# jjery2243542/adaptive_voice_conversion

Measured on NVIDIA H100. Metric: mel-segments/sec (80x128) train step, higher is better.
Workload: dtype tf32

## Files before the change

### adaptive_voice_conversion_b200/csrc/tc_common.cuh

```cuda
#pragma once
#include <cuda_runtime.h>
#include <stdint.h>

namespace avc {
namespace tc {

__device__ __forceinline__ uint32_t smem_u32(const void* p) { return (uint32_t)__cvta_generic_to_shared(p); }

__device__ __forceinline__ void mbar_init(uint64_t* bar, uint32_t count) {
  asm volatile("mbarrier.init.shared::cta.b64 [%0], %1;" ::"r"(smem_u32(bar)), "r"(count) : "memory");
}
__device__ __forceinline__ void fence_mbar_init() { asm volatile("fence.mbarrier_init.release.cluster;" ::: "memory"); }
__device__ __forceinline__ void mbar_arrive(uint64_t* bar) {
  asm volatile("mbarrier.arrive.shared::cta.b64 _, [%0];" ::"r"(smem_u32(bar)) : "memory");
}
__device__ __forceinline__ void mbar_arrive_expect_tx(uint64_t* bar, uint32_t bytes) {
  asm volatile("mbarrier.arrive.expect_tx.shared::cta.b64 _, [%0], %1;" ::"r"(smem_u32(bar)), "r"(bytes) : "memory");
}
__device__ __forceinline__ bool mbar_try_wait(uint64_t* bar, uint32_t parity) {
  uint32_t ok;
  asm volatile(
      "{\n\t.reg .pred p;\n\t"
      "mbarrier.try_wait.parity.shared::cta.b64 p, [%1], %2;\n\t"
      "selp.u32 %0, 1, 0, p;\n\t}"
// ... 45 lines not shown
}
__device__ __forceinline__ int warp_idx_sync() { return __shfl_sync(0xffffffffu, (int)(threadIdx.x >> 5), 0); }

template <int R>
__device__ __forceinline__ void setmaxnreg_dec() { asm volatile("setmaxnreg.dec.sync.aligned.u32 %0;" ::"n"(R)); }
template <int R>
__device__ __forceinline__ void setmaxnreg_inc() { asm volatile("setmaxnreg.inc.sync.aligned.u32 %0;" ::"n"(R)); }

__device__ __forceinline__ void wgmma_fence() { asm volatile("wgmma.fence.sync.aligned;" ::: "memory"); }
__device__ __forceinline__ void wgmma_commit() { asm volatile("wgmma.commit_group.sync.aligned;" ::: "memory"); }
template <int N>
__device__ __forceinline__ void wgmma_wait() { asm volatile("wgmma.wait_group.sync.aligned %0;" ::"n"(N) : "memory"); }
__device__ __forceinline__ void acc_fence(float* d, int n) {
  for (int i = 0; i < n; ++i) asm volatile("" : "+f"(d[i])::"memory");
}

template <int N>
__device__ __forceinline__ void wgmma_tf32(float* d, uint64_t a, uint64_t b, uint32_t acc);
template <> __device__ __forceinline__ void wgmma_tf32<16>(float* d, uint64_t a, uint64_t b, uint32_t acc) {
  asm volatile("{\n\t.reg .pred p;\n\tsetp.ne.b32 p, %10, 0;\n\t"
               "wgmma.mma_async.sync.aligned.m64n16k8.f32.tf32.tf32 {%0, %1, %2, %3, %4, %5, %6, %7}, %8, %9, p, 1, 1;\n\t}"
               : "+f"(d[0]), "+f"(d[1]), "+f"(d[2]), "+f"(d[3]), "+f"(d[4]), "+f"(d[5]), "+f"(d[6]), "+f"(d[7])
               : "l"(a), "l"(b), "r"(acc));
}
template <> __device__ __forceinline__ void wgmma_tf32<32>(float* d, uint64_t a, uint64_t b, uint32_t acc) {
  asm volatile("{\n\t.reg .pred p;\n\tsetp.ne.b32 p, %18, 0;\n\t"
               "wgmma.mma_async.sync.aligned.m64n32k8.f32.tf32.tf32 {%0, %1, %2, %3, %4, %5, %6, %7, %8, %9, %10, %11, %12, %13, %14, %15}, %16, %17, p, 1, 1;\n\t}"
               : "+f"(d[0]), "+f"(d[1]), "+f"(d[2]), "+f"(d[3]), "+f"(d[4]), "+f"(d[5]), "+f"(d[6]), "+f"(d[7]), "+f"(d[8]), "+f"(d[9]), "+f"(d[10]), "+f"(d[11]), "+f"(d[12]), "+f"(d[13]), "+f"(d[14]), "+f"(d[15])
               : "l"(a), "l"(b), "r"(acc));
}
// ... 70 lines not shown
               : "l"(a), "l"(b), "r"(acc));
}
template <> __device__ __forceinline__ void wgmma_tf32<240>(float* d, uint64_t a, uint64_t b, uint32_t acc) {
  asm volatile("{\n\t.reg .pred p;\n\tsetp.ne.b32 p, %122, 0;\n\t"
               "wgmma.mma_async.sync.aligned.m64n240k8.f32.tf32.tf32 {%0, %1, %2, %3, %4, %5, %6, %7, %8, %9, %10, %11, %12, %13, %14, %15, %16, %17, %18, %19, %20, %21, %22, %23, %24, %25, %26, %27, %28, %29, %30, %31, %32, %33, %34, %35, %36, %37, %38, %39, %40, %41, %42, %43, %44, %45, %46, %47, %48, %49, %50, %51, %52, %53, %54, %55, %56, %57, %58, %59, %60, %61, %62, %63, %64, %65, %66, %67, %68, %69, %70, %71, %72, %73, %74, %75, %76, %77, %78, %79, %80, %81, %82, %83, %84, %85, %86, %87, %88, %89, %90, %91, %92, %93, %94, %95, %96, %97, %98, %99, %100, %101, %102, %103, %104, %105, %106, %107, %108, %109, %110, %111, %112, %113, %114, %115, %116, %117, %118, %119}, %120, %121, p, 1, 1;\n\t}"
               : "+f"(d[0]), "+f"(d[1]), "+f"(d[2]), "+f"(d[3]), "+f"(d[4]), "+f"(d[5]), "+f"(d[6]), "+f"(d[7]), "+f"(d[8]), "+f"(d[9]), "+f"(d[10]), "+f"(d[11]), "+f"(d[12]), "+f"(d[13]), "+f"(d[14]), "+f"(d[15]), "+f"(d[16]), "+f"(d[17]), "+f"(d[18]), "+f"(d[19]), "+f"(d[20]), "+f"(d[21]), "+f"(d[22]), "+f"(d[23]), "+f"(d[24]), "+f"(d[25]), "+f"(d[26]), "+f"(d[27]), "+f"(d[28]), "+f"(d[29]), "+f"(d[30]), "+f"(d[31]), "+f"(d[32]), "+f"(d[33]), "+f"(d[34]), "+f"(d[35]), "+f"(d[36]), "+f"(d[37]), "+f"(d[38]), "+f"(d[39]), "+f"(d[40]), "+f"(d[41]), "+f"(d[42]), "+f"(d[43]), "+f"(d[44]), "+f"(d[45]), "+f"(d[46]), "+f"(d[47]), "+f"(d[48]), "+f"(d[49]), "+f"(d[50]), "+f"(d[51]), "+f"(d[52]), "+f"(d[53]), "+f"(d[54]), "+f"(d[55]), "+f"(d[56]), "+f"(d[57]), "+f"(d[58]), "+f"(d[59]), "+f"(d[60]), "+f"(d[61]), "+f"(d[62]), "+f"(d[63]), "+f"(d[64]), "+f"(d[65]), "+f"(d[66]), "+f"(d[67]), "+f"(d[68]), "+f"(d[69]), "+f"(d[70]), "+f"(d[71]), "+f"(d[72]), "+f"(d[73]), "+f"(d[74]), "+f"(d[75]), "+f"(d[76]), "+f"(d[77]), "+f"(d[78]), "+f"(d[79]), "+f"(d[80]), "+f"(d[81]), "+f"(d[82]), "+f"(d[83]), "+f"(d[84]), "+f"(d[85]), "+f"(d[86]), "+f"(d[87]), "+f"(d[88]), "+f"(d[89]), "+f"(d[90]), "+f"(d[91]), "+f"(d[92]), "+f"(d[93]), "+f"(d[94]), "+f"(d[95]), "+f"(d[96]), "+f"(d[97]), "+f"(d[98]), "+f"(d[99]), "+f"(d[100]), "+f"(d[101]), "+f"(d[102]), "+f"(d[103]), "+f"(d[104]), "+f"(d[105]), "+f"(d[106]), "+f"(d[107]), "+f"(d[108]), "+f"(d[109]), "+f"(d[110]), "+f"(d[111]), "+f"(d[112]), "+f"(d[113]), "+f"(d[114]), "+f"(d[115]), "+f"(d[116]), "+f"(d[117]), "+f"(d[118]), "+f"(d[119])
               : "l"(a), "l"(b), "r"(acc));
}
template <> __device__ __forceinline__ void wgmma_tf32<256>(float* d, uint64_t a, uint64_t b, uint32_t acc) {
  asm volatile("{\n\t.reg .pred p;\n\tsetp.ne.b32 p, %130, 0;\n\t"
               "wgmma.mma_async.sync.aligned.m64n256k8.f32.tf32.tf32 {%0, %1, %2, %3, %4, %5, %6, %7, %8, %9, %10, %11, %12, %13, %14, %15, %16, %17, %18, %19, %20, %21, %22, %23, %24, %25, %26, %27, %28, %29, %30, %31, %32, %33, %34, %35, %36, %37, %38, %39, %40, %41, %42, %43, %44, %45, %46, %47, %48, %49, %50, %51, %52, %53, %54, %55, %56, %57, %58, %59, %60, %61, %62, %63, %64, %65, %66, %67, %68, %69, %70, %71, %72, %73, %74, %75, %76, %77, %78, %79, %80, %81, %82, %83, %84, %85, %86, %87, %88, %89, %90, %91, %92, %93, %94, %95, %96, %97, %98, %99, %100, %101, %102, %103, %104, %105, %106, %107, %108, %109, %110, %111, %112, %113, %114, %115, %116, %117, %118, %119, %120, %121, %122, %123, %124, %125, %126, %127}, %128, %129, p, 1, 1;\n\t}"
               : "+f"(d[0]), "+f"(d[1]), "+f"(d[2]), "+f"(d[3]), "+f"(d[4]), "+f"(d[5]), "+f"(d[6]), "+f"(d[7]), "+f"(d[8]), "+f"(d[9]), "+f"(d[10]), "+f"(d[11]), "+f"(d[12]), "+f"(d[13]), "+f"(d[14]), "+f"(d[15]), "+f"(d[16]), "+f"(d[17]), "+f"(d[18]), "+f"(d[19]), "+f"(d[20]), "+f"(d[21]), "+f"(d[22]), "+f"(d[23]), "+f"(d[24]), "+f"(d[25]), "+f"(d[26]), "+f"(d[27]), "+f"(d[28]), "+f"(d[29]), "+f"(d[30]), "+f"(d[31]), "+f"(d[32]), "+f"(d[33]), "+f"(d[34]), "+f"(d[35]), "+f"(d[36]), "+f"(d[37]), "+f"(d[38]), "+f"(d[39]), "+f"(d[40]), "+f"(d[41]), "+f"(d[42]), "+f"(d[43]), "+f"(d[44]), "+f"(d[45]), "+f"(d[46]), "+f"(d[47]), "+f"(d[48]), "+f"(d[49]), "+f"(d[50]), "+f"(d[51]), "+f"(d[52]), "+f"(d[53]), "+f"(d[54]), "+f"(d[55]), "+f"(d[56]), "+f"(d[57]), "+f"(d[58]), "+f"(d[59]), "+f"(d[60]), "+f"(d[61]), "+f"(d[62]), "+f"(d[63]), "+f"(d[64]), "+f"(d[65]), "+f"(d[66]), "+f"(d[67]), "+f"(d[68]), "+f"(d[69]), "+f"(d[70]), "+f"(d[71]), "+f"(d[72]), "+f"(d[73]), "+f"(d[74]), "+f"(d[75]), "+f"(d[76]), "+f"(d[77]), "+f"(d[78]), "+f"(d[79]), "+f"(d[80]), "+f"(d[81]), "+f"(d[82]), "+f"(d[83]), "+f"(d[84]), "+f"(d[85]), "+f"(d[86]), "+f"(d[87]), "+f"(d[88]), "+f"(d[89]), "+f"(d[90]), "+f"(d[91]), "+f"(d[92]), "+f"(d[93]), "+f"(d[94]), "+f"(d[95]), "+f"(d[96]), "+f"(d[97]), "+f"(d[98]), "+f"(d[99]), "+f"(d[100]), "+f"(d[101]), "+f"(d[102]), "+f"(d[103]), "+f"(d[104]), "+f"(d[105]), "+f"(d[106]), "+f"(d[107]), "+f"(d[108]), "+f"(d[109]), "+f"(d[110]), "+f"(d[111]), "+f"(d[112]), "+f"(d[113]), "+f"(d[114]), "+f"(d[115]), "+f"(d[116]), "+f"(d[117]), "+f"(d[118]), "+f"(d[119]), "+f"(d[120]), "+f"(d[121]), "+f"(d[122]), "+f"(d[123]), "+f"(d[124]), "+f"(d[125]), "+f"(d[126]), "+f"(d[127])
               : "l"(a), "l"(b), "r"(acc));
}

__device__ __forceinline__ int wg_acc_row(int t, int i) { return 16 * (t >> 5) + ((t & 31) >> 2) + ((i & 2) ? 8 : 0); }
__device__ __forceinline__ int wg_acc_col(int t, int i) { return 8 * (i >> 2) + 2 * (t & 3) + (i & 1); }

}
}
```

### adaptive_voice_conversion_b200/csrc/wgrad_tc.cu

```cuda
#include "common.cuh"
#include "tc_common.cuh"

namespace avc {

constexpr int WT_NT = 32;
constexpr int WG_ROWS = 32;
constexpr int WG_A_BYTES = (WG_ROWS / 4) * 128 * 16;
constexpr int WG_MAX_STAGES = 8;
constexpr int WG_SMEM_MAX = 224 * 1024;

struct WgTcArgs {
  avc_wgrad_desc d;
  float* scratch;
  int nslices, samp_per_slice, nstage, coutp;
  int* status;
};

__device__ __forceinline__ float comp4(const float4& v, int c) { return c == 0 ? v.x : c == 1 ? v.y : c == 2 ? v.z : v.w; }

struct WgJob {
  float4 v[4];
  uint32_t dst;
  int rot;
};

template <int K>
__device__ __forceinline__ WgJob wgrad_job_load(const WgTcArgs& a, int e, int ch, int b0, int R) {
  const avc_wgrad_desc& d = a.d;
  const int T = d.Tout;
  WgJob J;
  const bool is_dc = e < 256;
  const int f = is_dc ? e : e - 256;
  const int c4 = is_dc ? (f & 31) : (f & 7), pl = is_dc ? (f >> 5) : ((f >> 3) & 7), j = is_dc ? 0 : (f >> 6);
  const int r = ch * WG_ROWS + 4 * pl;
  const int g = r / T, t = r - g * T;
  J.rot = (c4 >> 1) & 3;
  if (is_dc) {
    J.dst = (uint32_t)pl * (128u * 16u) + (uint32_t)(4 * c4) * 16u;
    const int co = blockIdx.y * 128 + 4 * c4;
    if (r < R && co < d.Cout) {
      const float* src = d.dc + (size_t)(b0 + g) * d.dc_bstride + ((size_t)(co >> 2) * T + t) * 4;
#pragma unroll
      for (int i = 0; i < 4; ++i) J.v[i] = ldg4(src + 4 * i);
    } else {
#pragma unroll
      for (int i = 0; i < 4; ++i) J.v[i] = zero4();
    }
  } else {
    J.dst = (uint32_t)WG_A_BYTES + (uint32_t)pl * (uint32_t)(K * WT_NT * 16) + (uint32_t)(j * WT_NT + 4 * c4) * 16u;
    const int ci = blockIdx.x * WT_NT + 4 * c4;
    const bool v = r < R && ci < d.Cin;
    const float* col = d.x + (size_t)(v ? b0 + g : 0) * d.x_bstride + (size_t)((v ? ci : 0) >> 2) * d.Tin * 4;
#pragma unroll
    for (int i = 0; i < 4; ++i) {
      const int p = src_pos((t + i) * d.stride + j - d.pad_left, d.Tin, AVC_PAD_REFLECT, 1);
      J.v[i] = (v && p >= 0) ? ldg4(col + (size_t)p * 4) : zero4();
    }
  }
  return J;
}

__device__ __forceinline__ void wgrad_job_store(uint8_t* stage, const WgJob& J) {
#pragma unroll
  for (int k = 0; k < 4; ++k) {
    const int c = (k + J.rot) & 3;
    *reinterpret_cast<float4*>(stage + J.dst + (uint32_t)c * 16u) = make_float4(comp4(J.v[0], c), comp4(J.v[1], c), comp4(J.v[2], c), comp4(J.v[3], c));
  }
}

__host__ __device__ constexpr int wg_stagers(int K) { return K <= 5 ? 2 : 1; }
__host__ __device__ constexpr int wg_threads(int K) { return 128 * (wg_stagers(K) + 2); }

template <int K, bool ATOMIC>
__global__ void __launch_bounds__(wg_threads(K), 1) conv_wgrad_wgmma_kernel(const WgTcArgs a) {
  constexpr int STAGERS = wg_stagers(K);
  constexpr int N = K * WT_NT;
  constexpr uint32_t B_PLANE = N * 16;
  extern __shared__ __align__(1024) uint8_t smem[];
  __shared__ uint64_t bar_full[WG_MAX_STAGES], bar_empty[WG_MAX_STAGES];
  const avc_wgrad_desc& d = a.d;
  const int tid = threadIdx.x, warp = tc::warp_idx_sync(), lane = tid & 31;
  const int sl = blockIdx.z, b0 = sl * a.samp_per_slice;
  const int R = max(0, min(a.samp_per_slice, d.B - b0)) * d.Tout;
  const int nchunk = cdiv(R, WG_ROWS);
  const uint32_t stage_bytes = (uint32_t)WG_A_BYTES + 8u * B_PLANE;

  if (tid == 0) {
    for (int s = 0; s < a.nstage; ++s) {
      tc::mbar_init(&bar_full[s], 4);
      tc::mbar_init(&bar_empty[s], 2);
    }
    tc::fence_mbar_init();
  }
  __syncthreads();

  if (warp < 4 * STAGERS) {
    constexpr int NJOBS = 256 + 64 * K, JPT = (NJOBS + 127) / 128;
    const int stid = tid & 127;
    for (int ch = warp >> 2; ch < nchunk; ch += STAGERS) {
      const int s = ch % a.nstage;
      const uint32_t ph = (uint32_t)(ch / a.nstage) & 1u;
      WgJob J[JPT];
#pragma unroll
      for (int q = 0; q < JPT; ++q)
        if (stid + 128 * q < NJOBS) J[q] = wgrad_job_load<K>(a, stid + 128 * q, ch, b0, R);
      if (ch >= a.nstage && !__all_sync(0xffffffffu, tc::mbar_wait(&bar_empty[s], ph ^ 1u, a.status, 5))) return;
      uint8_t* stage = smem + (size_t)s * stage_bytes;
#pragma unroll
      for (int q = 0; q < JPT; ++q)
        if (stid + 128 * q < NJOBS) wgrad_job_store(stage, J[q]);
      tc::fence_proxy_async_smem();
      __syncwarp();
      if (lane == 0) tc::mbar_arrive(&bar_full[s]);
    }
    return;
  }

  const int wg = (warp >> 2) - STAGERS, wt = tid & 127;
  float acc[N / 2];
#pragma unroll
  for (int i = 0; i < N / 2; ++i) acc[i] = 0.f;
  const uint32_t smem0 = tc::smem_u32(smem), d_hi = tc::sdesc_hi(128);
  int s = 0, s_prev = -1;
  uint32_t ph = 0;
  tc::acc_fence(acc, N / 2);
  for (int ch = 0; ch < nchunk; ++ch) {
    if (!__all_sync(0xffffffffu, tc::mbar_wait(&bar_full[s], ph, a.status, 6))) {
      tc::wgmma_wait<0>();
      return;
    }
    const uint32_t sw = smem0 + (uint32_t)s * stage_bytes;
    const uint32_t a_lo = tc::sdesc_lo(sw + (uint32_t)wg * 1024u, 128u * 16u), b_lo = tc::sdesc_lo(sw + (uint32_t)WG_A_BYTES, B_PLANE);
    tc::wgmma_fence();
#pragma unroll
    for (int k = 0; k < WG_ROWS / 8; ++k)
      tc::wgmma_tf32<N>(acc, tc::sdesc64(a_lo + (uint32_t)k * ((2u * 128u * 16u) >> 4), d_hi),
                        tc::sdesc64(b_lo + (uint32_t)k * ((2u * B_PLANE) >> 4), d_hi), 1u);
    tc::wgmma_commit();
    tc::wgmma_wait<1>();
    tc::acc_fence(acc, N / 2);
    if (s_prev >= 0 && wt == 0) tc::mbar_arrive(&bar_empty[s_prev]);
    s_prev = s;
    if (++s == a.nstage) { s = 0; ph ^= 1u; }
  }
  tc::wgmma_wait<0>();
  tc::acc_fence(acc, N / 2);
  if (nchunk == 0) return;

  const int co = blockIdx.y * 128 + 64 * wg + tc::wg_acc_row(wt, 0);
#pragma unroll
  for (int jj = 0; jj < N / 8; ++jj) {
    const int n = tc::wg_acc_col(wt, 4 * jj), j = n / WT_NT, ci = blockIdx.x * WT_NT + n % WT_NT;
    if (ci < d.Cin) {
      float* sbase = a.scratch + (((size_t)(ATOMIC ? 0 : sl) * K + j) * (size_t)(d.Cin >> 2)) * (size_t)a.coutp * 4;
#pragma unroll
      for (int h = 0; h < 2; ++h) {
        float* p = sbase + ((size_t)(ci >> 2) * a.coutp + co + 8 * h) * 4 + (ci & 3);
        const float v0 = acc[4 * jj + 2 * h], v1 = acc[4 * jj + 2 * h + 1];
        if constexpr (ATOMIC)
          asm volatile("red.global.add.v2.f32 [%0], {%1, %2};" ::"l"(p), "f"(v0), "f"(v1) : "memory");
        else
          *reinterpret_cast<float2*>(p) = make_float2(v0, v1);
      }
    }
// ... 88 lines not shown
}

static bool wgrad_tc_supported(const avc_wgrad_desc* d) {
  return (d->stride == 1 || d->stride == 2) && d->Tout % 8 == 0 && d->Tout <= 128 && d->K >= 1 && d->K <= 8 && d->Cin % 4 == 0 &&
         d->Cout % 4 == 0 && d->Tin + d->K - 1 >= (d->Tout - 1) * d->stride + 1 && (d->stride == 1 || d->Tout <= 64);
}

int wgrad_reduce(const float* scratch, float* dw, int Cout, int Cin, int K, int coutp, int nslices, cudaStream_t stream) {
  const int64_t n = (int64_t)K * (Cin / 4) * coutp;
  AVC_LAUNCH(wgrad_tc_reduce_kernel, (int)cdiv64(n, 32), dim3(32, 8), 0, stream, scratch, dw, Cout, Cin, K, coutp, nslices);
  AVC_CHECK_LAUNCH("wgrad_tc_reduce");
  return AVC_OK;
}

template <int K, bool ATOMIC>
static int wgrad_wgmma_launch(const WgTcArgs& a, cudaStream_t stream, const char* who) {
  static bool attr_done = false;
  if (!attr_done) {
    const cudaError_t e = cudaFuncSetAttribute(conv_wgrad_wgmma_kernel<K, ATOMIC>, cudaFuncAttributeMaxDynamicSharedMemorySize, WG_SMEM_MAX);
    if (e != cudaSuccess) {
      set_error("%s: cudaFuncSetAttribute: %s", who, cudaGetErrorString(e));
      return AVC_ERR_CUDA;
    }
    attr_done = true;
  }
  const dim3 grid(cdiv(a.d.Cin, WT_NT), cdiv(a.d.Cout, 128), a.nslices);
  const int smem = a.nstage * (WG_A_BYTES + 8 * 16 * WT_NT * K);
  AVC_LAUNCH((conv_wgrad_wgmma_kernel<K, ATOMIC>), grid, wg_threads(K), smem, stream, a);
  AVC_CHECK_LAUNCH(who);
  return AVC_OK;
}

template <bool ATOMIC>
static int wgrad_wgmma_dispatch(const WgTcArgs& a, cudaStream_t stream, const char* who) {
  switch (a.d.K) {
    case 1: return wgrad_wgmma_launch<1, ATOMIC>(a, stream, who);
    case 2: return wgrad_wgmma_launch<2, ATOMIC>(a, stream, who);
    case 3: return wgrad_wgmma_launch<3, ATOMIC>(a, stream, who);
    case 4: return wgrad_wgmma_launch<4, ATOMIC>(a, stream, who);
    case 5: return wgrad_wgmma_launch<5, ATOMIC>(a, stream, who);
    case 6: return wgrad_wgmma_launch<6, ATOMIC>(a, stream, who);
    case 7: return wgrad_wgmma_launch<7, ATOMIC>(a, stream, who);
    default: return wgrad_wgmma_launch<8, ATOMIC>(a, stream, who);
  }
}

}

using namespace avc;

extern "C" int64_t avc_wgrad_tc_scratch_floats(const avc_wgrad_desc* d) {
  if (!d || !wgrad_tc_supported(d)) return -1;
  WgTcArgs a;
  wgrad_tc_plan(d, a);
  return (int64_t)a.nslices * d->K * d->Cin * a.coutp;
}

static int wgrad_tc_launch(const avc_wgrad_desc* d, float* scratch, int* status, void* stream, bool accumulate, const char* who) {
  AVC_REQUIRE(d && d->x && d->dc && scratch && status && (accumulate || d->dw), AVC_ERR_INVALID, "%s: null argument", who);
  AVC_REQUIRE(d->B > 0 && d->Cin > 0 && d->Cout > 0 && d->Tin > 0 && d->Tout > 0, AVC_ERR_INVALID, "%s: bad shape", who);
  AVC_REQUIRE(wgrad_tc_supported(d), AVC_ERR_UNSUPPORTED, "%s: needs stride 1 (Tout <= 128) or 2 (Tout <= 64), Tout %% 8 == 0, K <= 8", who);
  WgTcArgs a;
  wgrad_tc_plan(d, a);
  a.scratch = scratch;
  a.status = status;
  const int rc = accumulate ? wgrad_wgmma_dispatch<true>(a, (cudaStream_t)stream, who) : wgrad_wgmma_dispatch<false>(a, (cudaStream_t)stream, who);
  if (rc != AVC_OK || accumulate) return rc;
  return wgrad_reduce(scratch, d->dw, d->Cout, d->Cin, d->K, a.coutp, a.nslices, (cudaStream_t)stream);
}

extern "C" int avc_conv_wgrad_tc(const avc_wgrad_desc* d, float* scratch, int* status, void* stream) {
  return wgrad_tc_launch(d, scratch, status, stream, false, "avc_conv_wgrad_tc");
}

extern "C" int64_t avc_wgrad_acc_floats(int Cout, int Cin, int K) {
  if (Cout <= 0 || Cin <= 0 || K <= 0 || Cin % 4 != 0) return -1;
  return (int64_t)K * Cin * (cdiv(Cout, 128) * 128);
}
extern "C" int avc_conv_wgrad_tc_acc(const avc_wgrad_desc* d, float* acc, int* status, void* stream) {
  return wgrad_tc_launch(d, acc, status, stream, true, "avc_conv_wgrad_tc_acc");
}
// ... 8 lines not shown
```

Baseline: 33960.

## Load wgrad dc tile via TMA and feed A operand from registers

The weight-gradient kernel no longer has stager threads copy the dc (output-gradient) tile into shared memory. A single thread now issues TMA tensor loads for it against a tensor map encoded on the host. The MMA warpgroups read the A operand from shared memory into registers and issue register-sourced wgmma, double-buffering the fragments across chunks. setmaxnreg also shifts registers from stager warps to MMA warps. This is meant to cut stager load and store work and shared-memory traffic, at the cost of a per-call tensor-map encode, new alignment requirements on dc, and extra register pressure.

```diff
diff --git a/adaptive_voice_conversion_b200/csrc/tc_common.cuh b/adaptive_voice_conversion_b200/csrc/tc_common.cuh
--- a/adaptive_voice_conversion_b200/csrc/tc_common.cuh
+++ b/adaptive_voice_conversion_b200/csrc/tc_common.cuh
@@ -83,6 +83,9 @@
 __device__ __forceinline__ void acc_fence(float* d, int n) {
   for (int i = 0; i < n; ++i) asm volatile("" : "+f"(d[i])::"memory");
 }
+__device__ __forceinline__ void reg_fence(uint32_t* r, int n) {
+  for (int i = 0; i < n; ++i) asm volatile("" : "+r"(r[i])::"memory");
+}
 
 template <int N>
 __device__ __forceinline__ void wgmma_tf32(float* d, uint64_t a, uint64_t b, uint32_t acc);
@@ -183,6 +186,57 @@
                : "l"(a), "l"(b), "r"(acc));
 }
 
+template <int N>
+__device__ __forceinline__ void wgmma_tf32_rs(float* d, const uint32_t* a, uint64_t b, uint32_t acc);
+template <> __device__ __forceinline__ void wgmma_tf32_rs<32>(float* d, const uint32_t* a, uint64_t b, uint32_t acc) {
+  asm volatile("{\n\t.reg .pred p;\n\tsetp.ne.b32 p, %21, 0;\n\t"
+               "wgmma.mma_async.sync.aligned.m64n32k8.f32.tf32.tf32 {%0, %1, %2, %3, %4, %5, %6, %7, %8, %9, %10, %11, %12, %13, %14, %15}, {%16, %17, %18, %19}, %20, p, 1, 1;\n\t}"
+               : "+f"(d[0]), "+f"(d[1]), "+f"(d[2]), "+f"(d[3]), "+f"(d[4]), "+f"(d[5]), "+f"(d[6]), "+f"(d[7]), "+f"(d[8]), "+f"(d[9]), "+f"(d[10]), "+f"(d[11]), "+f"(d[12]), "+f"(d[13]), "+f"(d[14]), "+f"(d[15])
+               : "r"(a[0]), "r"(a[1]), "r"(a[2]), "r"(a[3]), "l"(b), "r"(acc));
+}
+template <> __device__ __forceinline__ void wgmma_tf32_rs<64>(float* d, const uint32_t* a, uint64_t b, uint32_t acc) {
+  asm volatile("{\n\t.reg .pred p;\n\tsetp.ne.b32 p, %37, 0;\n\t"
+               "wgmma.mma_async.sync.aligned.m64n64k8.f32.tf32.tf32 {%0, %1, %2, %3, %4, %5, %6, %7, %8, %9, %10, %11, %12, %13, %14, %15, %16, %17, %18, %19, %20, %21, %22, %23, %24, %25, %26, %27, %28, %29, %30, %31}, {%32, %33, %34, %35}, %36, p, 1, 1;\n\t}"
+               : "+f"(d[0]), "+f"(d[1]), "+f"(d[2]), "+f"(d[3]), "+f"(d[4]), "+f"(d[5]), "+f"(d[6]), "+f"(d[7]), "+f"(d[8]), "+f"(d[9]), "+f"(d[10]), "+f"(d[11]), "+f"(d[12]), "+f"(d[13]), "+f"(d[14]), "+f"(d[15]), "+f"(d[16]), "+f"(d[17]), "+f"(d[18]), "+f"(d[19]), "+f"(d[20]), "+f"(d[21]), "+f"(d[22]), "+f"(d[23]), "+f"(d[24]), "+f"(d[25]), "+f"(d[26]), "+f"(d[27]), "+f"(d[28]), "+f"(d[29]), "+f"(d[30]), "+f"(d[31])
+               : "r"(a[0]), "r"(a[1]), "r"(a[2]), "r"(a[3]), "l"(b), "r"(acc));
+}
+template <> __device__ __forceinline__ void wgmma_tf32_rs<96>(float* d, const uint32_t* a, uint64_t b, uint32_t acc) {
+  asm volatile("{\n\t.reg .pred p;\n\tsetp.ne.b32 p, %53, 0;\n\t"
+               "wgmma.mma_async.sync.aligned.m64n96k8.f32.tf32.tf32 {%0, %1, %2, %3, %4, %5, %6, %7, %8, %9, %10, %11, %12, %13, %14, %15, %16, %17, %18, %19, %20, %21, %22, %23, %24, %25, %26, %27, %28, %29, %30, %31, %32, %33, %34, %35, %36, %37, %38, %39, %40, %41, %42, %43, %44, %45, %46, %47}, {%48, %49, %50, %51}, %52, p, 1, 1;\n\t}"
+               : "+f"(d[0]), "+f"(d[1]), "+f"(d[2]), "+f"(d[3]), "+f"(d[4]), "+f"(d[5]), "+f"(d[6]), "+f"(d[7]), "+f"(d[8]), "+f"(d[9]), "+f"(d[10]), "+f"(d[11]), "+f"(d[12]), "+f"(d[13]), "+f"(d[14]), "+f"(d[15]), "+f"(d[16]), "+f"(d[17]), "+f"(d[18]), "+f"(d[19]), "+f"(d[20]), "+f"(d[21]), "+f"(d[22]), "+f"(d[23]), "+f"(d[24]), "+f"(d[25]), "+f"(d[26]), "+f"(d[27]), "+f"(d[28]), "+f"(d[29]), "+f"(d[30]), "+f"(d[31]), "+f"(d[32]), "+f"(d[33]), "+f"(d[34]), "+f"(d[35]), "+f"(d[36]), "+f"(d[37]), "+f"(d[38]), "+f"(d[39]), "+f"(d[40]), "+f"(d[41]), "+f"(d[42]), "+f"(d[43]), "+f"(d[44]), "+f"(d[45]), "+f"(d[46]), "+f"(d[47])
+               : "r"(a[0]), "r"(a[1]), "r"(a[2]), "r"(a[3]), "l"(b), "r"(acc));
+}
+template <> __device__ __forceinline__ void wgmma_tf32_rs<128>(float* d, const uint32_t* a, uint64_t b, uint32_t acc) {
+  asm volatile("{\n\t.reg .pred p;\n\tsetp.ne.b32 p, %69, 0;\n\t"
+               "wgmma.mma_async.sync.aligned.m64n128k8.f32.tf32.tf32 {%0, %1, %2, %3, %4, %5, %6, %7, %8, %9, %10, %11, %12, %13, %14, %15, %16, %17, %18, %19, %20, %21, %22, %23, %24, %25, %26, %27, %28, %29, %30, %31, %32, %33, %34, %35, %36, %37, %38, %39, %40, %41, %42, %43, %44, %45, %46, %47, %48, %49, %50, %51, %52, %53, %54, %55, %56, %57, %58, %59, %60, %61, %62, %63}, {%64, %65, %66, %67}, %68, p, 1, 1;\n\t}"
+               : "+f"(d[0]), "+f"(d[1]), "+f"(d[2]), "+f"(d[3]), "+f"(d[4]), "+f"(d[5]), "+f"(d[6]), "+f"(d[7]), "+f"(d[8]), "+f"(d[9]), "+f"(d[10]), "+f"(d[11]), "+f"(d[12]), "+f"(d[13]), "+f"(d[14]), "+f"(d[15]), "+f"(d[16]), "+f"(d[17]), "+f"(d[18]), "+f"(d[19]), "+f"(d[20]), "+f"(d[21]), "+f"(d[22]), "+f"(d[23]), "+f"(d[24]), "+f"(d[25]), "+f"(d[26]), "+f"(d[27]), "+f"(d[28]), "+f"(d[29]), "+f"(d[30]), "+f"(d[31]), "+f"(d[32]), "+f"(d[33]), "+f"(d[34]), "+f"(d[35]), "+f"(d[36]), "+f"(d[37]), "+f"(d[38]), "+f"(d[39]), "+f"(d[40]), "+f"(d[41]), "+f"(d[42]), "+f"(d[43]), "+f"(d[44]), "+f"(d[45]), "+f"(d[46]), "+f"(d[47]), "+f"(d[48]), "+f"(d[49]), "+f"(d[50]), "+f"(d[51]), "+f"(d[52]), "+f"(d[53]), "+f"(d[54]), "+f"(d[55]), "+f"(d[56]), "+f"(d[57]), "+f"(d[58]), "+f"(d[59]), "+f"(d[60]), "+f"(d[61]), "+f"(d[62]), "+f"(d[63])
+               : "r"(a[0]), "r"(a[1]), "r"(a[2]), "r"(a[3]), "l"(b), "r"(acc));
+}
+template <> __device__ __forceinline__ void wgmma_tf32_rs<160>(float* d, const uint32_t* a, uint64_t b, uint32_t acc) {
+  asm volatile("{\n\t.reg .pred p;\n\tsetp.ne.b32 p, %85, 0;\n\t"
+               "wgmma.mma_async.sync.aligned.m64n160k8.f32.tf32.tf32 {%0, %1, %2, %3, %4, %5, %6, %7, %8, %9, %10, %11, %12, %13, %14, %15, %16, %17, %18, %19, %20, %21, %22, %23, %24, %25, %26, %27, %28, %29, %30, %31, %32, %33, %34, %35, %36, %37, %38, %39, %40, %41, %42, %43, %44, %45, %46, %47, %48, %49, %50, %51, %52, %53, %54, %55, %56, %57, %58, %59, %60, %61, %62, %63, %64, %65, %66, %67, %68, %69, %70, %71, %72, %73, %74, %75, %76, %77, %78, %79}, {%80, %81, %82, %83}, %84, p, 1, 1;\n\t}"
+               : "+f"(d[0]), "+f"(d[1]), "+f"(d[2]), "+f"(d[3]), "+f"(d[4]), "+f"(d[5]), "+f"(d[6]), "+f"(d[7]), "+f"(d[8]), "+f"(d[9]), "+f"(d[10]), "+f"(d[11]), "+f"(d[12]), "+f"(d[13]), "+f"(d[14]), "+f"(d[15]), "+f"(d[16]), "+f"(d[17]), "+f"(d[18]), "+f"(d[19]), "+f"(d[20]), "+f"(d[21]), "+f"(d[22]), "+f"(d[23]), "+f"(d[24]), "+f"(d[25]), "+f"(d[26]), "+f"(d[27]), "+f"(d[28]), "+f"(d[29]), "+f"(d[30]), "+f"(d[31]), "+f"(d[32]), "+f"(d[33]), "+f"(d[34]), "+f"(d[35]), "+f"(d[36]), "+f"(d[37]), "+f"(d[38]), "+f"(d[39]), "+f"(d[40]), "+f"(d[41]), "+f"(d[42]), "+f"(d[43]), "+f"(d[44]), "+f"(d[45]), "+f"(d[46]), "+f"(d[47]), "+f"(d[48]), "+f"(d[49]), "+f"(d[50]), "+f"(d[51]), "+f"(d[52]), "+f"(d[53]), "+f"(d[54]), "+f"(d[55]), "+f"(d[56]), "+f"(d[57]), "+f"(d[58]), "+f"(d[59]), "+f"(d[60]), "+f"(d[61]), "+f"(d[62]), "+f"(d[63]), "+f"(d[64]), "+f"(d[65]), "+f"(d[66]), "+f"(d[67]), "+f"(d[68]), "+f"(d[69]), "+f"(d[70]), "+f"(d[71]), "+f"(d[72]), "+f"(d[73]), "+f"(d[74]), "+f"(d[75]), "+f"(d[76]), "+f"(d[77]), "+f"(d[78]), "+f"(d[79])
+               : "r"(a[0]), "r"(a[1]), "r"(a[2]), "r"(a[3]), "l"(b), "r"(acc));
+}
+template <> __device__ __forceinline__ void wgmma_tf32_rs<192>(float* d, const uint32_t* a, uint64_t b, uint32_t acc) {
+  asm volatile("{\n\t.reg .pred p;\n\tsetp.ne.b32 p, %101, 0;\n\t"
+               "wgmma.mma_async.sync.aligned.m64n192k8.f32.tf32.tf32 {%0, %1, %2, %3, %4, %5, %6, %7, %8, %9, %10, %11, %12, %13, %14, %15, %16, %17, %18, %19, %20, %21, %22, %23, %24, %25, %26, %27, %28, %29, %30, %31, %32, %33, %34, %35, %36, %37, %38, %39, %40, %41, %42, %43, %44, %45, %46, %47, %48, %49, %50, %51, %52, %53, %54, %55, %56, %57, %58, %59, %60, %61, %62, %63, %64, %65, %66, %67, %68, %69, %70, %71, %72, %73, %74, %75, %76, %77, %78, %79, %80, %81, %82, %83, %84, %85, %86, %87, %88, %89, %90, %91, %92, %93, %94, %95}, {%96, %97, %98, %99}, %100, p, 1, 1;\n\t}"
+               : "+f"(d[0]), "+f"(d[1]), "+f"(d[2]), "+f"(d[3]), "+f"(d[4]), "+f"(d[5]), "+f"(d[6]), "+f"(d[7]), "+f"(d[8]), "+f"(d[9]), "+f"(d[10]), "+f"(d[11]), "+f"(d[12]), "+f"(d[13]), "+f"(d[14]), "+f"(d[15]), "+f"(d[16]), "+f"(d[17]), "+f"(d[18]), "+f"(d[19]), "+f"(d[20]), "+f"(d[21]), "+f"(d[22]), "+f"(d[23]), "+f"(d[24]), "+f"(d[25]), "+f"(d[26]), "+f"(d[27]), "+f"(d[28]), "+f"(d[29]), "+f"(d[30]), "+f"(d[31]), "+f"(d[32]), "+f"(d[33]), "+f"(d[34]), "+f"(d[35]), "+f"(d[36]), "+f"(d[37]), "+f"(d[38]), "+f"(d[39]), "+f"(d[40]), "+f"(d[41]), "+f"(d[42]), "+f"(d[43]), "+f"(d[44]), "+f"(d[45]), "+f"(d[46]), "+f"(d[47]), "+f"(d[48]), "+f"(d[49]), "+f"(d[50]), "+f"(d[51]), "+f"(d[52]), "+f"(d[53]), "+f"(d[54]), "+f"(d[55]), "+f"(d[56]), "+f"(d[57]), "+f"(d[58]), "+f"(d[59]), "+f"(d[60]), "+f"(d[61]), "+f"(d[62]), "+f"(d[63]), "+f"(d[64]), "+f"(d[65]), "+f"(d[66]), "+f"(d[67]), "+f"(d[68]), "+f"(d[69]), "+f"(d[70]), "+f"(d[71]), "+f"(d[72]), "+f"(d[73]), "+f"(d[74]), "+f"(d[75]), "+f"(d[76]), "+f"(d[77]), "+f"(d[78]), "+f"(d[79]), "+f"(d[80]), "+f"(d[81]), "+f"(d[82]), "+f"(d[83]), "+f"(d[84]), "+f"(d[85]), "+f"(d[86]), "+f"(d[87]), "+f"(d[88]), "+f"(d[89]), "+f"(d[90]), "+f"(d[91]), "+f"(d[92]), "+f"(d[93]), "+f"(d[94]), "+f"(d[95])
+               : "r"(a[0]), "r"(a[1]), "r"(a[2]), "r"(a[3]), "l"(b), "r"(acc));
+}
+template <> __device__ __forceinline__ void wgmma_tf32_rs<224>(float* d, const uint32_t* a, uint64_t b, uint32_t acc) {
+  asm volatile("{\n\t.reg .pred p;\n\tsetp.ne.b32 p, %117, 0;\n\t"
+               "wgmma.mma_async.sync.aligned.m64n224k8.f32.tf32.tf32 {%0, %1, %2, %3, %4, %5, %6, %7, %8, %9, %10, %11, %12, %13, %14, %15, %16, %17, %18, %19, %20, %21, %22, %23, %24, %25, %26, %27, %28, %29, %30, %31, %32, %33, %34, %35, %36, %37, %38, %39, %40, %41, %42, %43, %44, %45, %46, %47, %48, %49, %50, %51, %52, %53, %54, %55, %56, %57, %58, %59, %60, %61, %62, %63, %64, %65, %66, %67, %68, %69, %70, %71, %72, %73, %74, %75, %76, %77, %78, %79, %80, %81, %82, %83, %84, %85, %86, %87, %88, %89, %90, %91, %92, %93, %94, %95, %96, %97, %98, %99, %100, %101, %102, %103, %104, %105, %106, %107, %108, %109, %110, %111}, {%112, %113, %114, %115}, %116, p, 1, 1;\n\t}"
+               : "+f"(d[0]), "+f"(d[1]), "+f"(d[2]), "+f"(d[3]), "+f"(d[4]), "+f"(d[5]), "+f"(d[6]), "+f"(d[7]), "+f"(d[8]), "+f"(d[9]), "+f"(d[10]), "+f"(d[11]), "+f"(d[12]), "+f"(d[13]), "+f"(d[14]), "+f"(d[15]), "+f"(d[16]), "+f"(d[17]), "+f"(d[18]), "+f"(d[19]), "+f"(d[20]), "+f"(d[21]), "+f"(d[22]), "+f"(d[23]), "+f"(d[24]), "+f"(d[25]), "+f"(d[26]), "+f"(d[27]), "+f"(d[28]), "+f"(d[29]), "+f"(d[30]), "+f"(d[31]), "+f"(d[32]), "+f"(d[33]), "+f"(d[34]), "+f"(d[35]), "+f"(d[36]), "+f"(d[37]), "+f"(d[38]), "+f"(d[39]), "+f"(d[40]), "+f"(d[41]), "+f"(d[42]), "+f"(d[43]), "+f"(d[44]), "+f"(d[45]), "+f"(d[46]), "+f"(d[47]), "+f"(d[48]), "+f"(d[49]), "+f"(d[50]), "+f"(d[51]), "+f"(d[52]), "+f"(d[53]), "+f"(d[54]), "+f"(d[55]), "+f"(d[56]), "+f"(d[57]), "+f"(d[58]), "+f"(d[59]), "+f"(d[60]), "+f"(d[61]), "+f"(d[62]), "+f"(d[63]), "+f"(d[64]), "+f"(d[65]), "+f"(d[66]), "+f"(d[67]), "+f"(d[68]), "+f"(d[69]), "+f"(d[70]), "+f"(d[71]), "+f"(d[72]), "+f"(d[73]), "+f"(d[74]), "+f"(d[75]), "+f"(d[76]), "+f"(d[77]), "+f"(d[78]), "+f"(d[79]), "+f"(d[80]), "+f"(d[81]), "+f"(d[82]), "+f"(d[83]), "+f"(d[84]), "+f"(d[85]), "+f"(d[86]), "+f"(d[87]), "+f"(d[88]), "+f"(d[89]), "+f"(d[90]), "+f"(d[91]), "+f"(d[92]), "+f"(d[93]), "+f"(d[94]), "+f"(d[95]), "+f"(d[96]), "+f"(d[97]), "+f"(d[98]), "+f"(d[99]), "+f"(d[100]), "+f"(d[101]), "+f"(d[102]), "+f"(d[103]), "+f"(d[104]), "+f"(d[105]), "+f"(d[106]), "+f"(d[107]), "+f"(d[108]), "+f"(d[109]), "+f"(d[110]), "+f"(d[111])
+               : "r"(a[0]), "r"(a[1]), "r"(a[2]), "r"(a[3]), "l"(b), "r"(acc));
+}
+template <> __device__ __forceinline__ void wgmma_tf32_rs<256>(float* d, const uint32_t* a, uint64_t b, uint32_t acc) {
+  asm volatile("{\n\t.reg .pred p;\n\tsetp.ne.b32 p, %133, 0;\n\t"
+               "wgmma.mma_async.sync.aligned.m64n256k8.f32.tf32.tf32 {%0, %1, %2, %3, %4, %5, %6, %7, %8, %9, %10, %11, %12, %13, %14, %15, %16, %17, %18, %19, %20, %21, %22, %23, %24, %25, %26, %27, %28, %29, %30, %31, %32, %33, %34, %35, %36, %37, %38, %39, %40, %41, %42, %43, %44, %45, %46, %47, %48, %49, %50, %51, %52, %53, %54, %55, %56, %57, %58, %59, %60, %61, %62, %63, %64, %65, %66, %67, %68, %69, %70, %71, %72, %73, %74, %75, %76, %77, %78, %79, %80, %81, %82, %83, %84, %85, %86, %87, %88, %89, %90, %91, %92, %93, %94, %95, %96, %97, %98, %99, %100, %101, %102, %103, %104, %105, %106, %107, %108, %109, %110, %111, %112, %113, %114, %115, %116, %117, %118, %119, %120, %121, %122, %123, %124, %125, %126, %127}, {%128, %129, %130, %131}, %132, p, 1, 1;\n\t}"
+               : "+f"(d[0]), "+f"(d[1]), "+f"(d[2]), "+f"(d[3]), "+f"(d[4]), "+f"(d[5]), "+f"(d[6]), "+f"(d[7]), "+f"(d[8]), "+f"(d[9]), "+f"(d[10]), "+f"(d[11]), "+f"(d[12]), "+f"(d[13]), "+f"(d[14]), "+f"(d[15]), "+f"(d[16]), "+f"(d[17]), "+f"(d[18]), "+f"(d[19]), "+f"(d[20]), "+f"(d[21]), "+f"(d[22]), "+f"(d[23]), "+f"(d[24]), "+f"(d[25]), "+f"(d[26]), "+f"(d[27]), "+f"(d[28]), "+f"(d[29]), "+f"(d[30]), "+f"(d[31]), "+f"(d[32]), "+f"(d[33]), "+f"(d[34]), "+f"(d[35]), "+f"(d[36]), "+f"(d[37]), "+f"(d[38]), "+f"(d[39]), "+f"(d[40]), "+f"(d[41]), "+f"(d[42]), "+f"(d[43]), "+f"(d[44]), "+f"(d[45]), "+f"(d[46]), "+f"(d[47]), "+f"(d[48]), "+f"(d[49]), "+f"(d[50]), "+f"(d[51]), "+f"(d[52]), "+f"(d[53]), "+f"(d[54]), "+f"(d[55]), "+f"(d[56]), "+f"(d[57]), "+f"(d[58]), "+f"(d[59]), "+f"(d[60]), "+f"(d[61]), "+f"(d[62]), "+f"(d[63]), "+f"(d[64]), "+f"(d[65]), "+f"(d[66]), "+f"(d[67]), "+f"(d[68]), "+f"(d[69]), "+f"(d[70]), "+f"(d[71]), "+f"(d[72]), "+f"(d[73]), "+f"(d[74]), "+f"(d[75]), "+f"(d[76]), "+f"(d[77]), "+f"(d[78]), "+f"(d[79]), "+f"(d[80]), "+f"(d[81]), "+f"(d[82]), "+f"(d[83]), "+f"(d[84]), "+f"(d[85]), "+f"(d[86]), "+f"(d[87]), "+f"(d[88]), "+f"(d[89]), "+f"(d[90]), "+f"(d[91]), "+f"(d[92]), "+f"(d[93]), "+f"(d[94]), "+f"(d[95]), "+f"(d[96]), "+f"(d[97]), "+f"(d[98]), "+f"(d[99]), "+f"(d[100]), "+f"(d[101]), "+f"(d[102]), "+f"(d[103]), "+f"(d[104]), "+f"(d[105]), "+f"(d[106]), "+f"(d[107]), "+f"(d[108]), "+f"(d[109]), "+f"(d[110]), "+f"(d[111]), "+f"(d[112]), "+f"(d[113]), "+f"(d[114]), "+f"(d[115]), "+f"(d[116]), "+f"(d[117]), "+f"(d[118]), "+f"(d[119]), "+f"(d[120]), "+f"(d[121]), "+f"(d[122]), "+f"(d[123]), "+f"(d[124]), "+f"(d[125]), "+f"(d[126]), "+f"(d[127])
+               : "r"(a[0]), "r"(a[1]), "r"(a[2]), "r"(a[3]), "l"(b), "r"(acc));
+}
+
 __device__ __forceinline__ int wg_acc_row(int t, int i) { return 16 * (t >> 5) + ((t & 31) >> 2) + ((i & 2) ? 8 : 0); }
 __device__ __forceinline__ int wg_acc_col(int t, int i) { return 8 * (i >> 2) + 2 * (t & 3) + (i & 1); }
 
diff --git a/adaptive_voice_conversion_b200/csrc/wgrad_tc.cu b/adaptive_voice_conversion_b200/csrc/wgrad_tc.cu
--- a/adaptive_voice_conversion_b200/csrc/wgrad_tc.cu
+++ b/adaptive_voice_conversion_b200/csrc/wgrad_tc.cu
@@ -1,11 +1,13 @@
 #include "common.cuh"
 #include "tc_common.cuh"
+#include "tmap.cuh"
 
 namespace avc {
 
 constexpr int WT_NT = 32;
 constexpr int WG_ROWS = 32;
-constexpr int WG_A_BYTES = (WG_ROWS / 4) * 128 * 16;
+constexpr int WG_A_PLANE = 32 * 4 * 16;
+constexpr int WG_A_BYTES = (WG_ROWS / 4) * WG_A_PLANE;
 constexpr int WG_MAX_STAGES = 8;
 constexpr int WG_SMEM_MAX = 224 * 1024;
 
@@ -29,33 +31,18 @@
   const avc_wgrad_desc& d = a.d;
   const int T = d.Tout;
   WgJob J;
-  const bool is_dc = e < 256;
-  const int f = is_dc ? e : e - 256;
-  const int c4 = is_dc ? (f & 31) : (f & 7), pl = is_dc ? (f >> 5) : ((f >> 3) & 7), j = is_dc ? 0 : (f >> 6);
+  const int c4 = e & 7, pl = (e >> 3) & 7, j = e >> 6;
   const int r = ch * WG_ROWS + 4 * pl;
   const int g = r / T, t = r - g * T;
   J.rot = (c4 >> 1) & 3;
-  if (is_dc) {
-    J.dst = (uint32_t)pl * (128u * 16u) + (uint32_t)(4 * c4) * 16u;
-    const int co = blockIdx.y * 128 + 4 * c4;
-    if (r < R && co < d.Cout) {
-      const float* src = d.dc + (size_t)(b0 + g) * d.dc_bstride + ((size_t)(co >> 2) * T + t) * 4;
-#pragma unroll
-      for (int i = 0; i < 4; ++i) J.v[i] = ldg4(src + 4 * i);
-    } else {
-#pragma unroll
-      for (int i = 0; i < 4; ++i) J.v[i] = zero4();
-    }
-  } else {
-    J.dst = (uint32_t)WG_A_BYTES + (uint32_t)pl * (uint32_t)(K * WT_NT * 16) + (uint32_t)(j * WT_NT + 4 * c4) * 16u;
-    const int ci = blockIdx.x * WT_NT + 4 * c4;
-    const bool v = r < R && ci < d.Cin;
-    const float* col = d.x + (size_t)(v ? b0 + g : 0) * d.x_bstride + (size_t)((v ? ci : 0) >> 2) * d.Tin * 4;
-#pragma unroll
-    for (int i = 0; i < 4; ++i) {
-      const int p = src_pos((t + i) * d.stride + j - d.pad_left, d.Tin, AVC_PAD_REFLECT, 1);
-      J.v[i] = (v && p >= 0) ? ldg4(col + (size_t)p * 4) : zero4();
-    }
+  J.dst = (uint32_t)WG_A_BYTES + (uint32_t)pl * (uint32_t)(K * WT_NT * 16) + (uint32_t)(j * WT_NT + 4 * c4) * 16u;
+  const int ci = blockIdx.x * WT_NT + 4 * c4;
+  const bool v = r < R && ci < d.Cin;
+  const float* col = d.x + (size_t)(v ? b0 + g : 0) * d.x_bstride + (size_t)((v ? ci : 0) >> 2) * d.Tin * 4;
+#pragma unroll
+  for (int i = 0; i < 4; ++i) {
+    const int p = src_pos((t + i) * d.stride + j - d.pad_left, d.Tin, AVC_PAD_REFLECT, 1);
+    J.v[i] = (v && p >= 0) ? ldg4(col + (size_t)p * 4) : zero4();
   }
   return J;
 }
@@ -68,11 +55,39 @@
   }
 }
 
-__host__ __device__ constexpr int wg_stagers(int K) { return K <= 5 ? 2 : 1; }
+__host__ __device__ constexpr int wg_stagers(int K) { return K <= 6 ? 2 : 1; }
 __host__ __device__ constexpr int wg_threads(int K) { return 128 * (wg_stagers(K) + 2); }
+__host__ __device__ constexpr int wg_regs_stage(int K) { return wg_stagers(K) == 2 ? 96 : 104; }
+__host__ __device__ constexpr int wg_regs_mma(int K) { return wg_stagers(K) == 2 ? 160 : 200; }
+static_assert(2 * 128 * wg_regs_stage(1) + 256 * wg_regs_mma(1) <= 512 * 128 && 128 * wg_regs_stage(8) + 256 * wg_regs_mma(8) <= 384 * 168,
+              "setmaxnreg budget exceeds the launch allocation");
+
+template <int N>
+__device__ __forceinline__ bool wgrad_mma_stage(const WgTcArgs& a, float* acc, uint32_t* af, uint32_t* af_prev, uint64_t* full, int s, uint32_t ph,
+                                                const uint8_t* stage, uint32_t a_off, uint32_t b_lo, uint32_t d_hi) {
+  constexpr uint32_t B_PLANE = N * 16;
+  if (!__all_sync(0xffffffffu, tc::mbar_wait(&full[s], ph, a.status, 6))) {
+    tc::wgmma_wait<0>();
+    return false;
+  }
+#pragma unroll
+  for (int k = 0; k < WG_ROWS / 8; ++k)
+#pragma unroll
+    for (int q = 0; q < 4; ++q)
+      af[4 * k + q] = *reinterpret_cast<const uint32_t*>(stage + a_off + (uint32_t)(2 * k + (q >> 1)) * WG_A_PLANE + (uint32_t)(q & 1) * 128u);
+  tc::wgmma_fence();
+#pragma unroll
+  for (int k = 0; k < WG_ROWS / 8; ++k)
+    tc::wgmma_tf32_rs<N>(acc, af + 4 * k, tc::sdesc64(b_lo + (uint32_t)k * ((2u * B_PLANE) >> 4), d_hi), 1u);
+  tc::wgmma_commit();
+  tc::wgmma_wait<1>();
+  tc::acc_fence(acc, N / 2);
+  tc::reg_fence(af_prev, 16);
+  return true;
+}
 
 template <int K, bool ATOMIC>
-__global__ void __launch_bounds__(wg_threads(K), 1) conv_wgrad_wgmma_kernel(const WgTcArgs a) {
+__global__ void __launch_bounds__(wg_threads(K), 1) conv_wgrad_wgmma_kernel(const WgTcArgs a, const __grid_constant__ CUtensorMap tmdc) {
   constexpr int STAGERS = wg_stagers(K);
   constexpr int N = K * WT_NT;
   constexpr uint32_t B_PLANE = N * 16;
@@ -87,7 +102,7 @@
 
   if (tid == 0) {
     for (int s = 0; s < a.nstage; ++s) {
-      tc::mbar_init(&bar_full[s], 4);
+      tc::mbar_init(&bar_full[s], 5);
       tc::mbar_init(&bar_empty[s], 2);
     }
     tc::fence_mbar_init();
@@ -95,7 +110,8 @@
   __syncthreads();
 
   if (warp < 4 * STAGERS) {
-    constexpr int NJOBS = 256 + 64 * K, JPT = (NJOBS + 127) / 128;
+    tc::setmaxnreg_dec<wg_regs_stage(K)>();
+    constexpr int NJOBS = 64 * K, JPT = (NJOBS + 127) / 128;
     const int stid = tid & 127;
     for (int ch = warp >> 2; ch < nchunk; ch += STAGERS) {
       const int s = ch % a.nstage;
@@ -106,6 +122,14 @@
         if (stid + 128 * q < NJOBS) J[q] = wgrad_job_load<K>(a, stid + 128 * q, ch, b0, R);
       if (ch >= a.nstage && !__all_sync(0xffffffffu, tc::mbar_wait(&bar_empty[s], ph ^ 1u, a.status, 5))) return;
       uint8_t* stage = smem + (size_t)s * stage_bytes;
+      if (stid == 0) {
+        tc::mbar_arrive_expect_tx(&bar_full[s], (uint32_t)WG_A_BYTES);
+#pragma unroll
+        for (int p = 0; p < WG_ROWS / 4; ++p) {
+          const int r = ch * WG_ROWS + 4 * p, g = r / d.Tout;
+          tc::tensor_g2s_4d(stage + p * WG_A_PLANE, &tmdc, 0, r - g * d.Tout, blockIdx.y * 32, r < R ? b0 + g : d.B, &bar_full[s]);
+        }
+      }
 #pragma unroll
       for (int q = 0; q < JPT; ++q)
         if (stid + 128 * q < NJOBS) wgrad_job_store(stage, J[q]);
@@ -116,38 +140,35 @@
     return;
   }
 
+  tc::setmaxnreg_inc<wg_regs_mma(K)>();
   const int wg = (warp >> 2) - STAGERS, wt = tid & 127;
   float acc[N / 2];
 #pragma unroll
   for (int i = 0; i < N / 2; ++i) acc[i] = 0.f;
+  const int m = 64 * wg + tc::wg_acc_row(wt, 0);
+  const uint32_t a_off = (uint32_t)(m >> 2) * 64u + (uint32_t)(wt & 3) * 16u + (uint32_t)(m & 3) * 4u;
+  uint32_t af[2][16];
   const uint32_t smem0 = tc::smem_u32(smem), d_hi = tc::sdesc_hi(128);
   int s = 0, s_prev = -1;
   uint32_t ph = 0;
   tc::acc_fence(acc, N / 2);
   for (int ch = 0; ch < nchunk; ++ch) {
-    if (!__all_sync(0xffffffffu, tc::mbar_wait(&bar_full[s], ph, a.status, 6))) {
-      tc::wgmma_wait<0>();
-      return;
-    }
-    const uint32_t sw = smem0 + (uint32_t)s * stage_bytes;
-    const uint32_t a_lo = tc::sdesc_lo(sw + (uint32_t)wg * 1024u, 128u * 16u), b_lo = tc::sdesc_lo(sw + (uint32_t)WG_A_BYTES, B_PLANE);
-    tc::wgmma_fence();
-#pragma unroll
-    for (int k = 0; k < WG_ROWS / 8; ++k)
-      tc::wgmma_tf32<N>(acc, tc::sdesc64(a_lo + (uint32_t)k * ((2u * 128u * 16u) >> 4), d_hi),
-                        tc::sdesc64(b_lo + (uint32_t)k * ((2u * B_PLANE) >> 4), d_hi), 1u);
-    tc::wgmma_commit();
-    tc::wgmma_wait<1>();
-    tc::acc_fence(acc, N / 2);
+    const uint32_t b_lo = tc::sdesc_lo(smem0 + (uint32_t)s * stage_bytes + (uint32_t)WG_A_BYTES, B_PLANE);
+    const uint8_t* stage = smem + (size_t)s * stage_bytes;
+    const bool ok = (ch & 1) ? wgrad_mma_stage<N>(a, acc, af[1], af[0], bar_full, s, ph, stage, a_off, b_lo, d_hi)
+                             : wgrad_mma_stage<N>(a, acc, af[0], af[1], bar_full, s, ph, stage, a_off, b_lo, d_hi);
+    if (!ok) return;
     if (s_prev >= 0 && wt == 0) tc::mbar_arrive(&bar_empty[s_prev]);
     s_prev = s;
     if (++s == a.nstage) { s = 0; ph ^= 1u; }
   }
   tc::wgmma_wait<0>();
   tc::acc_fence(acc, N / 2);
+  tc::reg_fence(af[0], 16);
+  tc::reg_fence(af[1], 16);
   if (nchunk == 0) return;
 
-  const int co = blockIdx.y * 128 + 64 * wg + tc::wg_acc_row(wt, 0);
+  const int co = blockIdx.y * 128 + m;
 #pragma unroll
   for (int jj = 0; jj < N / 8; ++jj) {
     const int n = tc::wg_acc_col(wt, 4 * jj), j = n / WT_NT, ci = blockIdx.x * WT_NT + n % WT_NT;
@@ -266,7 +287,7 @@
 }
 
 template <int K, bool ATOMIC>
-static int wgrad_wgmma_launch(const WgTcArgs& a, cudaStream_t stream, const char* who) {
+static int wgrad_wgmma_launch(const WgTcArgs& a, const CUtensorMap& tmdc, cudaStream_t stream, const char* who) {
   static bool attr_done = false;
   if (!attr_done) {
     const cudaError_t e = cudaFuncSetAttribute(conv_wgrad_wgmma_kernel<K, ATOMIC>, cudaFuncAttributeMaxDynamicSharedMemorySize, WG_SMEM_MAX);
@@ -278,22 +299,22 @@
   }
   const dim3 grid(cdiv(a.d.Cin, WT_NT), cdiv(a.d.Cout, 128), a.nslices);
   const int smem = a.nstage * (WG_A_BYTES + 8 * 16 * WT_NT * K);
-  AVC_LAUNCH((conv_wgrad_wgmma_kernel<K, ATOMIC>), grid, wg_threads(K), smem, stream, a);
+  AVC_LAUNCH((conv_wgrad_wgmma_kernel<K, ATOMIC>), grid, wg_threads(K), smem, stream, a, tmdc);
   AVC_CHECK_LAUNCH(who);
   return AVC_OK;
 }
 
 template <bool ATOMIC>
-static int wgrad_wgmma_dispatch(const WgTcArgs& a, cudaStream_t stream, const char* who) {
+static int wgrad_wgmma_dispatch(const WgTcArgs& a, const CUtensorMap& tmdc, cudaStream_t stream, const char* who) {
   switch (a.d.K) {
-    case 1: return wgrad_wgmma_launch<1, ATOMIC>(a, stream, who);
-    case 2: return wgrad_wgmma_launch<2, ATOMIC>(a, stream, who);
-    case 3: return wgrad_wgmma_launch<3, ATOMIC>(a, stream, who);
-    case 4: return wgrad_wgmma_launch<4, ATOMIC>(a, stream, who);
-    case 5: return wgrad_wgmma_launch<5, ATOMIC>(a, stream, who);
-    case 6: return wgrad_wgmma_launch<6, ATOMIC>(a, stream, who);
-    case 7: return wgrad_wgmma_launch<7, ATOMIC>(a, stream, who);
-    default: return wgrad_wgmma_launch<8, ATOMIC>(a, stream, who);
+    case 1: return wgrad_wgmma_launch<1, ATOMIC>(a, tmdc, stream, who);
+    case 2: return wgrad_wgmma_launch<2, ATOMIC>(a, tmdc, stream, who);
+    case 3: return wgrad_wgmma_launch<3, ATOMIC>(a, tmdc, stream, who);
+    case 4: return wgrad_wgmma_launch<4, ATOMIC>(a, tmdc, stream, who);
+    case 5: return wgrad_wgmma_launch<5, ATOMIC>(a, tmdc, stream, who);
+    case 6: return wgrad_wgmma_launch<6, ATOMIC>(a, tmdc, stream, who);
+    case 7: return wgrad_wgmma_launch<7, ATOMIC>(a, tmdc, stream, who);
+    default: return wgrad_wgmma_launch<8, ATOMIC>(a, tmdc, stream, who);
   }
 }
 
@@ -312,11 +333,27 @@
   AVC_REQUIRE(d && d->x && d->dc && scratch && status && (accumulate || d->dw), AVC_ERR_INVALID, "%s: null argument", who);
   AVC_REQUIRE(d->B > 0 && d->Cin > 0 && d->Cout > 0 && d->Tin > 0 && d->Tout > 0, AVC_ERR_INVALID, "%s: bad shape", who);
   AVC_REQUIRE(wgrad_tc_supported(d), AVC_ERR_UNSUPPORTED, "%s: needs stride 1 (Tout <= 128) or 2 (Tout <= 64), Tout %% 8 == 0, K <= 8", who);
+  AVC_REQUIRE(((uintptr_t)d->dc & 15u) == 0 && d->dc_bstride % 4 == 0, AVC_ERR_UNSUPPORTED,
+              "%s: dc and its sample stride (%lld floats) must be 16-byte aligned", who, (long long)d->dc_bstride);
   WgTcArgs a;
   wgrad_tc_plan(d, a);
   a.scratch = scratch;
   a.status = status;
-  const int rc = accumulate ? wgrad_wgmma_dispatch<true>(a, (cudaStream_t)stream, who) : wgrad_wgmma_dispatch<false>(a, (cudaStream_t)stream, who);
+  CUtensorMap tmdc;
+  {
+    PFN_tmap_encode enc = tmap_encode_fn();
+    AVC_REQUIRE(enc, AVC_ERR_CUDA, "%s: cuTensorMapEncodeTiled is not available from this driver", who);
+    const cuuint64_t gdim[4] = {4, (cuuint64_t)d->Tout, (cuuint64_t)(d->Cout / 4), (cuuint64_t)d->B};
+    const cuuint64_t gstr[3] = {16, (cuuint64_t)d->Tout * 16u, (cuuint64_t)d->dc_bstride * 4u};
+    const cuuint32_t box[4] = {4, 4, 32, 1};
+    const cuuint32_t estr[4] = {1, 1, 1, 1};
+    const CUresult r = enc(&tmdc, CU_TENSOR_MAP_DATA_TYPE_FLOAT32, 4, (void*)d->dc, gdim, gstr, box, estr, CU_TENSOR_MAP_INTERLEAVE_NONE,
+                           CU_TENSOR_MAP_SWIZZLE_NONE, CU_TENSOR_MAP_L2_PROMOTION_L2_256B, CU_TENSOR_MAP_FLOAT_OOB_FILL_NONE);
+    AVC_REQUIRE(r == CUDA_SUCCESS, AVC_ERR_CUDA, "%s: cuTensorMapEncodeTiled failed (%d) for dc: B=%d Cout=%d Tout=%d bstride=%lld", who, (int)r,
+                d->B, d->Cout, d->Tout, (long long)d->dc_bstride);
+  }
+  const int rc = accumulate ? wgrad_wgmma_dispatch<true>(a, tmdc, (cudaStream_t)stream, who)
+                            : wgrad_wgmma_dispatch<false>(a, tmdc, (cudaStream_t)stream, who);
   if (rc != AVC_OK || accumulate) return rc;
   return wgrad_reduce(scratch, d->dw, d->Cout, d->Cin, d->K, a.coutp, a.nslices, (cudaStream_t)stream);
 }
```

Result: faster. 36090, median of 6 (+6.3%).
